# VachaLab/gorder

Hardware: AMD Instinct MI355X
Metric: trajectory frames/sec (higher is better)
Workload: dtype f32

## Files before the change

gorder_amd/csrc/gorder_hip.hip:

```cpp
#include <hip/hip_runtime.h>

#include <dlfcn.h>

#include <cmath>
#include <cstdio>
#include <cstdlib>
#include <cstring>
#include <mutex>
#include <new>
#include <string>
#include <deque>
#include <type_traits>
#include <vector>

#include "../../include/gorder_hip.h"
#include "gm_math.h"
#include "plan.h"
#include "collect_store.h"
#include "device_mem.h"
#include "replay_rows.h"
#include "leaflet_rows.h"
#include "timewise_blocks.h"
#include "ordermap_final.h"
#include "order_route.h"
// ... 107 lines not shown
    uint32_t rows_frames = 0;
    RepAcc acc;
    size_t lds_bytes = 0;
    bool direct = false;
    bool force_direct = false;
    uint32_t forced_subrange = 0;
    uint64_t row_bytes = gorder::kClassRowBytes;
    bool on() const { return n_classes != 0; }
};

struct gorder_hip_handle {
    void *traj_cache = nullptr;
    void (*traj_cache_free)(gorder_hip_handle *) = nullptr;
    Plan plan;
    gorder_tables_t tables{};
    int device = 0;
    Stream own_stream;
    hipStream_t stream = nullptr;
    DBuf<Tile> d_tiles;
    DBuf<Item> d_items;
    DBuf<uint32_t> d_tile_slots;
    DBuf<DirectItem> d_direct;
    DBuf<Tile> d_ua_tiles;
    DBuf<gorder::UaItem> d_ua_items;
    DBuf<uint32_t> d_ua_tile_slots;
    uint32_t map_nx = 0, map_ny = 0;
    DBuf<u64> d_map_sums, d_map_cnts;
    DBuf<u64> d_map_packed;
    DBuf<u64> d_map_rec;
    DBuf<gorder::MapRun> d_ua_runs, d_runs;
    DBuf<uint32_t> d_ua_run_begin, d_run_begin;
    DBuf<Item> d_items_by_slot;
    DBuf<uint32_t> d_ua_item_run, d_item_run;
    DBuf<uint4> d_lgrid;
    DBuf<LocalRowPre> d_lrowpre;
    DBuf<LocalEdge> d_ledge;
    DBuf<float4> d_lfinfo;
    static constexpr uint32_t kDecidePause = 16;
    DBuf<uint32_t> d_lsummary;
    HBuf<uint32_t> h_lsummary;
    Event lsummary_written;
    bool lsummary_pending = false;
    uint32_t decide_pause = 0;
    uint64_t decide_submits = 0, decide_paused_submits = 0;
    DBuf<uint32_t> d_lneed;
    DBuf<uint2> d_ltodo;
    size_t map_lds_bytes = 0;
    bool map_staged = false;
    uint64_t map_pending = 0;
    uint64_t map_fold_limit = kMapFoldLimit;
    uint32_t map_max_mol = 1;
    DBuf<u64> d_tw_sums, d_tw_cnts;
    uint64_t tw_cap = 0;
    DBuf<u64> d_twx_blocks, d_twx_rows, d_twx_totals, d_twx_edge;
    DBuf<uint32_t> d_twx_groups;
    DBuf<float> d_twx_out;
    DBuf<uint32_t> d_omx_groups;
    DBuf<float> d_omx_out;
    ExtraArgs extra{};
    DBuf<uint32_t> d_geom_group;
    DBuf<float> d_shapes;
    DBuf<float> d_inv_box;
    uint32_t dyn_slab = 4, local_slab = 4;
    bool local_halo = false;
    size_t local_rec_stride = 0;
    DBuf<XtcCheckpoint> d_xtc_cp;
// ... 536 lines not shown
                           b.aflags, b.arow, h->d_tiles, bond_items(h, s.route), h->d_tile_slots, nt);
    }); });
    return GORDER_OK;
}

int launch_dist(gorder_hip_handle *h, const SubRange &s, const ExtraArgs &e) {
    const uint32_t nt = (uint32_t)h->plan.tiles.size();
    const gorder::FrameChunks c = gorder::dist_chunks(s.nf(), nt, h->wg_target, h->wg_capacity, h->hist_direct ? 0u : (uint32_t)h->hist_table_words,
                                                      h->hist_samples_per_word, kDistChunkMax);
    FrameArgs b = s.frames(c);
    DistArgs da{};
    da.n_edges = h->hist_edges; da.edges = h->d_hist_edges; da.rep = h->hist.rep; da.n_rep = h->hist.n_rep;
    const size_t lds = kDistEdgeBytes + std::max<size_t>(kDistReduceBytes, h->hist_direct ? 0u : h->hist_table_words * sizeof(uint32_t));
    TIMING_MARK(h, s.route.label);
    with_bool(literal_cosine(h), [&](auto AC) { with_bool(h->hist_direct, [&](auto DIRECT) {
        hipLaunchKernelGGL((k_bonds_dist<AC(), DIRECT()>), dim3(nt * c.n_chunks), dim3(kBlock), lds, h->stream, b, e, da, b.xyz, b.box9,
                           b.aflags, b.arow, h->d_tiles, bond_items(h, s.route), h->d_tile_slots, nt);
    }); });
    return GORDER_OK;
}

int launch_extras(gorder_hip_handle *h, const SubRange &s, const ExtraArgs &e) {
    const uint32_t nt = (uint32_t)h->plan.tiles.size();
    const gorder::FrameChunks c = gorder::extras_chunks(s.nf(), nt, h->wg_target, h->wg_capacity, s.route.map_accumulate, false);
    FrameArgs b = s.frames(c);
    TIMING_MARK(h, s.route.label);
    with_bool(literal_cosine(h), [&](auto AC) { with_bool(s.route.maps_only, [&](auto MO) {
        hipLaunchKernelGGL((k_bonds_extras<AC(), MO()>), dim3(nt * c.n_chunks), dim3(kBlock), 0, h->stream, b, e, b.xyz, b.box9, b.aflags,
                           b.arow, h->d_tiles, bond_items(h, s.route), h->d_tile_slots, nt);
    }); });
    return GORDER_OK;
}

int launch_tiled_out(gorder_hip_handle *h, const SubRange &s, const ExtraArgs &e) {
    const gorder::OrderRoute &route = s.route;
    const uint32_t nt = (uint32_t)h->plan.tiles.size();
    const gorder::FrameChunks c = gorder::extras_chunks(s.nf(), nt, h->wg_target, h->wg_capacity, route.map_accumulate,
                                                        route.family == gorder::BondFamily::TiledTw);
    FrameArgs b = s.frames(c);
    const dim3 g(nt * c.n_chunks), blk(kBlock);
    const Item *items = bond_items(h, route);
    TIMING_MARK(h, route.label);
    with_npf(route.npf, [&](auto NPF) { with_bool(b.pbc, [&](auto PBC) { with_bool(b.leaflets, [&](auto LF) { with_axis(h->axis, [&](auto AX) {
        if (route.family == gorder::BondFamily::TiledMaps)
            hipLaunchKernelGGL((k_bonds_tiled_maps<NPF(), PBC(), LF(), AX()>), g, blk, h->lds_bytes, h->stream, b, e, b.xyz,
                               b.box9, b.aflags, b.arow, h->d_tiles, items, h->d_tile_slots, nt, h->lw);
        else with_bool(route.tw_maps, [&](auto MAPS) { with_bool(route.mom, [&](auto MOM) {
            if constexpr (!MOM() || (LF() && !MAPS()))
                hipLaunchKernelGGL((k_bonds_tiled_tw<NPF(), PBC(), LF(), AX(), MAPS(), MOM()>), g, blk, h->lds_bytes, h->stream, b, e,
                                   b.xyz, b.box9, b.aflags, b.arow, h->d_tiles, items, h->d_tile_slots, nt, h->lw);
        }); });
    }); }); }); });
    return GORDER_OK;
}

int launch_map_accumulate(gorder_hip_handle *h, const SubRange &s, uint32_t rec_stride, const gorder::MapRun *runs,
                          const uint32_t *run_begin, uint32_t per_item) {
    const uint32_t n_acc = h->plan.n_acc;
    const uint32_t planes = h->tables.leaflets.method != GORDER_LEAFLETS_NONE ? 2u : 1u;
    const uint32_t ntm = h->map_nx * h->map_ny, n_words = planes * ntm;
    const char *ev = getenv("GORDER_HIP_MAP_CHUNKS");
    const gorder::FrameChunks m = gorder::map_chunks(s.nf(), n_acc, ev ? (uint32_t)std::max(1, atoi(ev)) : 0u);
    TIMING_MARK(h, "k_map_accumulate");
    hipLaunchKernelGGL(k_map_accumulate, dim3(n_acc * m.n_chunks), dim3(1024), n_words * sizeof(unsigned long long), h->stream,
                       h->d_map_rec, runs, run_begin, n_acc, s.nf(), rec_stride, m.frames_per_chunk, per_item, n_words, ntm,
                       h->d_map_packed, n_acc);
    return GORDER_OK;
}

int launch_bond_pass(gorder_hip_handle *h, const SubRange &s, ExtraArgs &e) {
    using gorder::BondFamily;
    e.item_run = h->d_item_run;
    switch (s.route.family) {
    case BondFamily::Classes: ST_TRY(launch_classes(h, s)); break;
    case BondFamily::Shells: ST_TRY(launch_shells(h, s, e)); break;
    case BondFamily::Dist: ST_TRY(launch_dist(h, s, e)); break;
    case BondFamily::Extras: ST_TRY(launch_extras(h, s, e)); break;
    default: ST_TRY(launch_tiled_out(h, s, e)); break;
    }
    if (s.route.map_accumulate) ST_TRY(launch_map_accumulate(h, s, e.rec_stride, h->d_runs, h->d_run_begin, 1u));
    HIP_TRY(h, hipGetLastError());
    return GORDER_OK;
}

int launch_ua_dist(gorder_hip_handle *h, const SubRange &s, const ExtraArgs &e) {
    const uint32_t nt = (uint32_t)h->plan.ua_tiles.size();
    const gorder::FrameChunks c = gorder::dist_chunks(s.nf(), nt, h->wg_target, h->wg_capacity, h->hist_direct ? 0u : (uint32_t)h->hist_table_words,
                                                      h->hist_samples_per_word, kDistChunkMax);
    FrameArgs b = s.frames(c);
    DistArgs da{};
    da.n_edges = h->hist_edges; da.edges = h->d_hist_edges; da.rep = h->hist.rep; da.n_rep = h->hist.n_rep;
    const size_t lds = kDistEdgeBytes + std::max<size_t>(kUaSumBytes, h->hist_direct ? 0u : h->hist_table_words * sizeof(uint32_t));
    const dim3 g((uint32_t)ua_grid(nt, c.n_chunks)), blk(kBlock);
    TIMING_MARK(h, "k_ua_dist");
    with_bool(literal_cosine(h), [&](auto AC) { with_bool(h->hist_direct, [&](auto DIRECT) {
        hipLaunchKernelGGL((k_ua_dist<AC(), DIRECT()>), g, blk, lds, h->stream, b, e, da, b.xyz, b.box9, b.aflags, b.arow, h->d_ua_tiles,
                           h->d_ua_items, h->d_ua_tile_slots, nt);
    }); });
    HIP_TRY(h, hipGetLastError());
    return GORDER_OK;
}

int launch_ua_pass(gorder_hip_handle *h, const SubRange &s, ExtraArgs &e) {
    const gorder::OrderRoute &route = s.route;
    if (route.ua_kernel == gorder::UaKernel::Dist) return launch_ua_dist(h, s, e);
// ... 717 lines not shown
    h->tables = *t;
    h->tables.molecule_types = nullptr;
    h->tables.leaflets.membrane = nullptr;
    h->device = t->device;
    HIP_TRY(h, hipSetDevice(h->device));
    if ((t->flags & GORDER_FLAG_UA_FAST_NORMALISE) && (t->flags & GORDER_FLAG_TRIG_ACOS_COS))
        return fail(h, GORDER_ERR_INVALID_ARGUMENT, "GORDER_FLAG_UA_FAST_NORMALISE (tolerance-bounded) and GORDER_FLAG_TRIG_ACOS_COS (literal) exclude each other");
    if ((t->flags & GORDER_FLAG_CLUSTER_CUTOFF) && t->leaflets.method != GORDER_LEAFLETS_CLUSTERING)
        return fail(h, GORDER_ERR_INVALID_ARGUMENT, "GORDER_FLAG_CLUSTER_CUTOFF needs leaflets.method == GORDER_LEAFLETS_CLUSTERING");
    const bool ua_rows_only = t->timewise && !t->ordermap.enabled && t->geometry.kind == GORDER_GEOM_NONE && !t->dynamic_normal.enabled;
    const int st = gorder::build_plan(*t, env_flag("GORDER_HIP_FORCE_DIRECT"), h->plan, !env_flag("GORDER_HIP_UA_SLOT_WAVES") && !ua_rows_only);
    if (st != GORDER_OK) return fail(h, st, "invalid bond tables");
    const Plan &p = h->plan;
    for (uint32_t m = 0; m < t->n_molecule_types; m++)
        h->map_max_mol = std::max(h->map_max_mol, t->molecule_types[m].n_molecules);
    HIP_TRY(h, h->own_stream.create());
    h->stream = h->own_stream;
    ST_TRY(upload(h, h->d_tiles, p.tiles));
    ST_TRY(upload(h, h->d_items, p.items));
    ST_TRY(upload(h, h->d_tile_slots, p.tile_slots));
    ST_TRY(upload(h, h->d_direct, p.direct));
    ST_TRY(upload(h, h->d_ua_tiles, p.ua_tiles));
    ST_TRY(upload(h, h->d_ua_items, p.ua_items));
    ST_TRY(upload(h, h->d_ua_tile_slots, p.ua_tile_slots));
    ExtraArgs &e = h->extra;
    e.sin_tet = sinf(1.910633f); e.cos_tet = cosf(1.910633f);
    e.sin_ch3 = sinf(2.0943952f); e.cos_ch3 = cosf(2.0943952f);
    e.sin_half = sinf(0.9553165f); e.cos_half = cosf(0.9553165f);
    ST_TRY(create_ordermaps(h, t));
    e.tw = t->timewise ? 1 : 0;
    if (t->timewise && !p.tiles.empty()) {
        if (!h->d_items_by_slot) ST_TRY(upload(h, h->d_items_by_slot, p.items_by_slot));
        ST_TRY(upload(h, h->d_item_run, p.item_run));
    }
    ST_TRY(create_geometry(h, t));
    if ((e.maps || e.tw || e.geom_kind) && !p.direct.empty())
        return fail(h, GORDER_ERR_INVALID_ARGUMENT, "ordermaps / timewise / geometry need every bond to fit an atom window");
    ST_TRY(create_accumulators(h));
    {
        const float *n = t->normal;
        h->n2sq = (n[0] * n[0] + n[1] * n[1]) + n[2] * n[2];
        h->n2 = sqrtf(h->n2sq);
        for (int d = 0; d < 3; d++)
            if (n[d] == 1.0f && n[(d + 1) % 3] == 0.0f && n[(d + 2) % 3] == 0.0f) h->axis = d;
        h->extra.axis = h->axis;
    }
    if (const char *e = getenv("GORDER_HIP_KERNEL")) h->use_gather = strcmp(e, "gather") == 0;
    h->shell_force_direct = env_flag("GORDER_HIP_RADIAL_DIRECT");
    h->hist_force_direct = env_flag("GORDER_HIP_DIST_DIRECT");
    h->nb.force_direct = env_flag("GORDER_HIP_NB_DIRECT");
    if (const char *ev = getenv("GORDER_HIP_NB_SUBRANGE")) h->nb.forced_subrange = (uint32_t)std::max(0, atoi(ev));
    if (const char *ev = getenv("GORDER_HIP_NB_ROW_BYTES")) {
        const long long v = atoll(ev);
        if (v > 0) h->nb.row_bytes = (uint64_t)v;
    }
    if (const char *ev = getenv("GORDER_HIP_CORR_SUBRANGE")) h->corr.forced_subrange = (uint32_t)std::max(0, atoi(ev));
    if (const char *ev = getenv("GORDER_HIP_CORR_GRID")) h->corr.chunk_major = strcmp(ev, "chunks") == 0;
    if (const char *ev = getenv("GORDER_HIP_DIST_SAMPLES_PER_WORD")) h->hist_samples_per_word = (uint32_t)std::min(std::max(0, atoi(ev)), 1 << 16);
    if (const char *e = getenv("GORDER_HIP_MOL_ROWS_STAGING")) {
        const long long v = atoll(e);
        if (v > 0) h->mol_stage_bytes = (size_t)v;
    }
    if (const char *e = getenv("GORDER_HIP_WG_TARGET")) {
        const int w = atoi(e);
        if (w > 0) h->wg_target = (uint32_t)w;
    }
// ... 533 lines not shown
    ri.bond_tiles = !p.tiles.empty(); ri.ua_tiles = !p.ua_tiles.empty(); ri.direct_items = !p.direct.empty(); ri.ua_fast_flag = (h->tables.flags & GORDER_FLAG_UA_FAST_NORMALISE) != 0;
    ri.global_leaflets = h->tables.leaflets.method == GORDER_LEAFLETS_GLOBAL; ri.spec_enabled = h->spec_enabled && !h->corr.on(); ri.have_assignment = h->have_assignment;
    ri.shells = h->n_shells != 0;
    ri.dist = h->hist_edges != 0;
    ri.classes = h->nb.on();
    ri.mol_rows = h->mol.n_groups != 0 && !h->mol_failed;
    ri.ua_samples_flag = (h->tables.flags & GORDER_FLAG_UA_SAMPLES) != 0;
    ri.npf5 = env_flag("GORDER_HIP_NPF5"); ri.tw_gather = env_flag("GORDER_HIP_TW_GATHER"); ri.maps_gather = env_flag("GORDER_HIP_MAPS_GATHER");
    ri.every_frame_assigns = b.aframes.size() == b.n_frames;
    b.route = gorder::choose_order_route(ri);
    if (!b.route.speculative) return;
    spec_poll(h, false);
    const uint32_t slot = (uint32_t)(h->spec_batches % gorder_hip_handle::kSpecRing);
    if (h->spec_ring_frames[slot]) (void)hipEventSynchronize(h->spec_counters_copied[slot]), spec_poll(h, false);
    ri.spec_enabled = h->spec_enabled && !h->corr.on();
    if (!ri.spec_enabled) b.route = gorder::choose_order_route(ri);
}

static int fill_flag_rows(gorder_hip_handle *h, Batch &b) {
    if (!b.leaflets) return GORDER_OK;
    const bool spec = b.route.speculative;
    if (spec) std::fill(b.arow.begin(), b.arow.end(), 0u);
    const size_t rows = (b.ltable ? b.replay.expand.size() : b.aframes.size()) + 1;
    ST_TRY(ensure_flag_rows(h, rows, rows + rows / 4, true));
    ST_TRY(upload_if_changed(h, h->d_arow, h->up_arow, h->up_arow_valid, b.arow));
    if (h->collect & GORDER_COLLECT_LEAFLETS)
        for (uint32_t f : b.aframes) b.collect_frames.push_back(b.frame_index[f]);
    if (spec) b.spec_aframes = b.aframes;
    else if (b.ltable) BATCH_TRY(replay_flag_rows(h, b.replay));
    else BATCH_TRY(run_leaflets(h, b.d_xyz, b.d_box, b.aframes, 1));
    h->have_assignment = true;
    h->assignment_frame = b.last_assign_frame;
    b.n_new_rows = spec ? 0 : (b.ltable ? b.replay.expand.size() : b.aframes.size());
    return GORDER_OK;
}

static int grow_frame_rows(gorder_hip_handle *h, const Batch &b) {
    if (!h->extra.tw || h->n_frames + b.n_frames <= h->tw_cap) return GORDER_OK;
    const size_t row = 3 * (size_t)h->plan.n_acc;
    const uint64_t ncap = (h->n_frames + b.n_frames) * 2;
    DBuf<u64> ns, nc;
    ST_TRY(allocate(h, ns, ncap * row));
    ST_TRY(allocate(h, nc, ncap * row));
    HIP_TRY(h, hipMemsetAsync(ns, 0, ncap * row * sizeof(u64), h->stream));
    HIP_TRY(h, hipMemsetAsync(nc, 0, ncap * row * sizeof(u64), h->stream));
    if (h->d_tw_sums) {
        HIP_TRY(h, hipMemcpyAsync(ns, h->d_tw_sums, h->n_frames * row * sizeof(u64), hipMemcpyDeviceToDevice, h->stream));
        HIP_TRY(h, hipMemcpyAsync(nc, h->d_tw_cnts, h->n_frames * row * sizeof(u64), hipMemcpyDeviceToDevice, h->stream));
        HIP_TRY(h, hipStreamSynchronize(h->stream));
    }
    h->d_tw_sums.swap(ns); h->d_tw_cnts.swap(nc); h->tw_cap = ncap;
    return GORDER_OK;
}

static int set_batch_normals(gorder_hip_handle *h, Batch &b) {
    const Plan &p = h->plan;
    FrameArgs &a = b.a;
    a.xyz = b.d_xyz; a.box9 = b.d_box; a.n_atoms = p.n_atoms; a.n_frames = b.n_frames;
    a.pbc = b.pbc ? 1 : 0;
    a.nx = h->tables.normal[0]; a.ny = h->tables.normal[1]; a.nz = h->tables.normal[2]; a.n2 = h->n2; a.n2sq = h->n2sq;
    a.leaflets = b.leaflets ? 1 : 0; a.aflags = h->d_aflags; a.arow = h->d_arow; a.n_mol_total = p.n_mol_total;
    a.acc = h->d_acc; a.rep = h->d_rep; a.n_rep = h->n_rep; a.n_acc = p.n_acc; a.err = h->d_err;
    h->manual_active = false;
    if (h->manual_frames) {
        const size_t n4 = (size_t)b.n_frames * p.n_mol_total;
        BATCH_TRY(ensure(h, h->d_dyn_normals, n4));
// ... 1318 lines not shown
```

gorder_amd/csrc/kernels_extras.h:

```cpp
#pragma once

namespace {

struct ExtraArgs {
    int maps;
    uint32_t plane;
    float x0, y0, binx, biny;
    uint32_t nx, ny;
    unsigned long long *map_packed;
    unsigned long long *map_rec;
    const uint32_t *item_run;
    uint32_t rec_frame0, rec_stride;
    const float4 *dyn;
    int bin_core;
    float inv_binx, inv_biny;
    int axis;
    int tw;
    unsigned long long *tw_sums;
    unsigned long long *tw_cnts;
    unsigned long long tw_row0;
    float sin_tet, cos_tet, sin_ch3, cos_ch3, sin_half, cos_half;
    int geom_kind, geom_invert, geom_orient;
    float geom_thr;
    const float *shapes;
    const float *inv_box;
    uint8_t *touched;
};

__device__ __forceinline__ bool geom_inside(const ExtraArgs &e, const float *sh, float px, float py, float pz,
                                            const float *box, bool pbc, int &bad) {
    bool in = true;
    if (e.geom_kind == GORDER_GEOM_CUBOID) {
        float x = px - sh[0], y = py - sh[1], z = pz - sh[2];
        if (pbc) {
            x = gm_wrap(x, box[0], bad); y = gm_wrap(y, box[1], bad); z = gm_wrap(z, box[2], bad);
            in = (x <= sh[3]) && (y <= sh[4]) && (z <= sh[5]);
        } else {
            in = (x >= 0.0f) && (x <= sh[3]) && (y >= 0.0f) && (y <= sh[4]) && (z >= 0.0f) && (z <= sh[5]);
        }
    } else if (e.geom_kind == GORDER_GEOM_CYLINDER) {
        const int o = e.geom_orient;
        const float dx = px - sh[0], dy = py - sh[1], dz = pz - sh[2];
        float x = o == 0 ? dx : (o == 1 ? dy : dz), da = o == 0 ? dy : (o == 1 ? dz : dx), db = o == 0 ? dz : (o == 1 ? dx : dy);
        if (pbc) {
            const float bo = o == 0 ? box[0] : (o == 1 ? box[1] : box[2]), ba = o == 0 ? box[1] : (o == 1 ? box[2] : box[0]),
                        bb = o == 0 ? box[2] : (o == 1 ? box[0] : box[1]);
            da = gm_min_image(da, ba, bad); db = gm_min_image(db, bb, bad); x = gm_wrap(x, bo, bad);
        }
        in = (da * da + db * db < e.geom_thr) && (pbc ? true : (x >= 0.0f)) && (x <= sh[7]);
    } else {
        float dx = px - sh[0], dy = py - sh[1], dz = pz - sh[2];
        if (pbc) { dx = gm_min_image(dx, box[0], bad); dy = gm_min_image(dy, box[1], bad); dz = gm_min_image(dz, box[2], bad); }
        in = (dx * dx + dy * dy) + dz * dz < e.geom_thr;
// ... 220 lines not shown
        __syncthreads();
        if (f0 + G < f_full) S::template load<false>(a, t, f0 + G, f_end, sk, si, pre);
        if (active) S::template compute<1>(a, t, it, f0, lds, lw, acc, bad, nan_which, nan_frame, &mo);
        rec_store(e, tile_id, f0, tid, words);
        __syncthreads();
    }
    if (f_full < f_end) {
        S::template load<true>(a, t, f_full, f_end, sk, si, pre);
        S::template store<true>(a, t, f_full, f_end, sk, si, pre, lds, lw);
        __syncthreads();
#pragma unroll
        for (uint32_t m = 0; m < kRecFrames; m++) words[m] = kMapNoSample;
        if (active) S::template compute_tail<1>(a, t, it, f_full, f_end, lds, lw, acc, bad, nan_which, nan_frame, &mo);
        rec_store(e, tile_id, f_full, tid, words);
        __syncthreads();
    }
    raise_tile_errors(a.err, tc, tile_slots, nan_which, nan_frame, bad);
    __syncthreads();
    fold_tile_sums(a.rep, a.n_rep, a.n_acc, tc, acc, lds, [&] { return tile_slots[tc.t.slot0 + tc.tid]; });
}

template <int NPF, bool PBC, bool LEAF, int AXIS, bool MAPS, bool MOM = false>
__global__ __launch_bounds__(kBlock, 4) void k_bonds_tiled_tw(FrameArgs a_in, ExtraArgs e, const float *__restrict__ xyz,
                                                             const float *__restrict__ box9, const uint8_t *__restrict__ aflags,
                                                             const uint32_t *__restrict__ arow, const Tile *__restrict__ tiles,
                                                             const Item *__restrict__ items, const uint32_t *__restrict__ tile_slots,
                                                             uint32_t n_tiles, uint32_t lw) {
    constexpr int G = (int)kRecFrames;
    extern __shared__ __attribute__((aligned(16))) float lds[];
    __shared__ int l_tick[kRecFrames][kBlock];
    __shared__ uint8_t l_side[kRecFrames][kBlock];
    __shared__ uint32_t l_slot_run[kBlock];
    __shared__ uint32_t l_slot_id[kBlock];
    using S = TiledStage<G, NPF, false, PBC, LEAF, AXIS>;
    FrameArgs a = a_in;
    a.xyz = xyz; a.box9 = box9; a.aflags = aflags; a.arow = arow;
    const uint32_t tile_id = blockIdx.x % n_tiles, chunk = blockIdx.x / n_tiles;
    const Tile t = tiles[tile_id];
    const uint32_t tid = threadIdx.x;
    const uint32_t sk = tid / S::TPF, si = tid % S::TPF;
    const bool active = tid < t.n_items;
    Item it{0, 0, 0, 0, 0};
    if (active) {
        it = items[t.item0 + tid];
        const uint32_t run = e.item_run[t.item0 + tid];
        if ((run >> 16) == tid) l_slot_run[it.lslot] = run;
    }
    const uint32_t f_begin = a.frame0 + chunk * a.frames_per_chunk;
    const uint32_t f_end = min(a.n_frames, f_begin + a.frames_per_chunk);
    const TileCtx tc{t, it, tile_id, chunk, tid, active, f_begin, f_end};
    unsigned long long words[kRecFrames], mwords[MAPS ? kRecFrames : 1];
    TiledMapOut mo{};
    if (MAPS) {
        mo = tiled_map_out(e, mwords);
        mo.ticks = words;
    } else {
        mo.nx = 0;
        mo.words = words;
    }
    SampleAcc acc;
    int bad = 0;
    uint32_t nan_which = 0, nan_frame = kNoNan;
    v4f pre[NPF];
    const uint32_t my_slot = tid < t.n_slots ? tile_slots[t.slot0 + tid] : 0u;
    l_slot_id[tid] = my_slot;
    uint2 own = make_uint2(0u, 0u), my_head = make_uint2(0u, 0xffffffffu);
    if (MOM) {
        own = a.own[tile_id];
        const uint32_t hq = a.own_head_begin[tile_id] + (tid & 63u);
        if (hq < a.own_head_begin[tile_id + 1u]) my_head = a.own_heads[hq];
    }
    if (f_begin + G <= f_end) S::template load<false>(a, t, f_begin, f_end, sk, si, pre);
    for (uint32_t fs = f_begin; fs < f_end; fs += G) {
        const bool full = fs + G <= f_end;
        bool finite;
        if (full) {
            finite = S::template store<false, MOM>(a, t, fs, f_end, sk, si, pre, lds, lw);
        } else {
            S::template load<true>(a, t, fs, f_end, sk, si, pre);
            finite = S::template store<true, MOM>(a, t, fs, f_end, sk, si, pre, lds, lw);
        }
        __syncthreads();
        if (full && fs + 2u * G <= f_end) S::template load<false>(a, t, fs + G, f_end, sk, si, pre);
        if (MOM && fs + sk < f_end) {
            static_assert(!MOM || (uint32_t)G * 64u == kBlock, "a wave per frame slot");
            tiled_moments(a, t, own, tile_id, n_tiles, fs + sk, lds + (size_t)sk * lw, finite, my_head);
        }
#pragma unroll
        for (uint32_t k = 0; k < kRecFrames; k++) { words[k] = kMapNoSample; if (MAPS) mwords[k] = kMapNoSample; }
        if (active) {
            if (full) S::template compute<MAPS ? 3 : 2>(a, t, it, fs, lds, lw, acc, bad, nan_which, nan_frame, &mo);
            else S::template compute_tail<MAPS ? 3 : 2>(a, t, it, fs, f_end, lds, lw, acc, bad, nan_which, nan_frame, &mo);
        }
        if constexpr (MAPS) rec_store(e, tile_id, fs, tid, mwords);
#pragma unroll
        for (uint32_t k = 0; k < kRecFrames; k++) {
            l_tick[k][tid] = (int)(uint32_t)words[k];
            l_side[k][tid] = words[k] == kMapNoSample ? (uint8_t)2 : (uint8_t)(words[k] >> 32);
        }
        __syncthreads();
        for (uint32_t w = tid; w < kRecFrames * t.n_slots; w += kBlock) {
            const uint32_t k = w % kRecFrames, ls = w / kRecFrames;
            if (fs + k >= f_end) continue;
            const uint32_t run = l_slot_run[ls], tid0 = run >> 16, n = run & 0xffffu;
            int s_all = 0, s_low = 0;
            uint32_t n_all = 0, n_low = 0;
            for (uint32_t j = 0; j < n; j++) {
                const uint32_t side = l_side[k][tid0 + j];
                const int tick = l_tick[k][tid0 + j];
                if (side == 2u) continue;
                s_all += tick; n_all += 1u;
                if (side == 1u) { s_low += tick; n_low += 1u; }
            }
            if (!n_all) continue;
            const uint32_t slot = l_slot_id[ls];
            const size_t row = ((size_t)e.tw_row0 + fs + k) * 3u * a.n_acc;
            atomicAdd(&e.tw_sums[row + slot], (unsigned long long)(long long)s_all);
            atomicAdd(&e.tw_cnts[row + slot], (unsigned long long)n_all);
            if (LEAF) {
                const uint32_t n_up = n_all - n_low;
                if (n_up) {
                    atomicAdd(&e.tw_sums[row + (size_t)a.n_acc + slot], (unsigned long long)(long long)(s_all - s_low));
                    atomicAdd(&e.tw_cnts[row + (size_t)a.n_acc + slot], (unsigned long long)n_up);
                }
            }
        }
    }
    __syncthreads();
    raise_tile_errors(a.err, tc, tile_slots, nan_which, nan_frame, bad);
    fold_tile_sums(a.rep, a.n_rep, a.n_acc, tc, acc, lds, [&] { return my_slot; });
}

constexpr uint32_t kMapRunBatch = 1024;
__global__ __launch_bounds__(1024) void k_map_accumulate(const unsigned long long *__restrict__ rec,
                                                         const gorder::MapRun *__restrict__ runs,
                                                         const uint32_t *__restrict__ run_begin, uint32_t n_slots,
                                                         uint32_t rec_frames, uint32_t rec_stride,
                                                         uint32_t frames_per_chunk, uint32_t k_max,
                                                         uint32_t n_words , uint32_t n_tiles_map,
                                                         unsigned long long *__restrict__ map_packed, uint32_t n_acc) {
    extern __shared__ unsigned long long l_map[];
    typedef unsigned long long ull2 __attribute__((ext_vector_type(2)));
    const uint32_t slot = blockIdx.x % n_slots, chunk = blockIdx.x / n_slots;
    const uint32_t r0 = run_begin[slot], r1 = run_begin[slot + 1];
    if (r0 == r1) return;
    const uint32_t f0 = chunk * frames_per_chunk, f1 = min(rec_frames, f0 + frames_per_chunk);
    for (uint32_t w = threadIdx.x; w < n_words; w += blockDim.x) l_map[w] = 0ull;
    __syncthreads();
    auto add = [&](unsigned long long v) {
        if (v != kMapNoSample) atomicAdd(&l_map[(uint32_t)(v >> 32)], kMapOne + (unsigned long long)(long long)(int)(uint32_t)v);
    };
    if (k_max == 1u) {
        __shared__ uint32_t l_pref[kMapRunBatch + 1];
        const uint32_t fb0 = f0 / kRecFrames, fb1 = (f1 + kRecFrames - 1) / kRecFrames;
        for (uint32_t rb = r0; rb < r1; rb += kMapRunBatch) {
            const uint32_t nr = min(kMapRunBatch, r1 - rb);
            for (uint32_t i = threadIdx.x; i < nr; i += blockDim.x) l_pref[i + 1u] = runs[rb + i].n;
// ... 79 lines not shown
```

gorder_amd/csrc/kernels_timewise.h:

```cpp
#pragma once

using gorder::kTwChunkFrames;
typedef unsigned long long tw_u64;

__device__ __forceinline__ float tw_mean(tw_u64 sum, tw_u64 count) {
    const long long q = (long long)sum / (long long)count;
    return (float)((double)q / 1e6);
}

__global__ __launch_bounds__(256) void k_tw_blocks(const tw_u64 *__restrict__ tw_sums, const tw_u64 *__restrict__ tw_cnts,
                                                   uint32_t row_words, uint32_t fold_words, tw_u64 n_used, tw_u64 first_position,
                                                   tw_u64 block_size, tw_u64 *__restrict__ out_sums, tw_u64 *__restrict__ out_cnts) {
    const uint32_t j = blockIdx.y * blockDim.x + threadIdx.x;
    if (j >= fold_words) return;
    tw_u64 r = (tw_u64)blockIdx.x * kTwChunkFrames;
    const tw_u64 end = r + kTwChunkFrames < n_used ? r + kTwChunkFrames : n_used;
    while (r < end) {
        const tw_u64 b = gorder::tw_block_of(first_position, r, block_size);
        const tw_u64 e = gorder::tw_segment_end(first_position, r, end, b, block_size);
        tw_u64 s = 0, c = 0;
        for (tw_u64 q = r; q < e; q++) {
            s += tw_sums[q * row_words + j];
            c += tw_cnts[q * row_words + j];
        }
        atomicAdd(&out_sums[b * row_words + j], s);
        atomicAdd(&out_cnts[b * row_words + j], c);
        r = e;
    }
}

__global__ __launch_bounds__(256) void k_tw_lower(tw_u64 *__restrict__ sums, tw_u64 *__restrict__ cnts, uint32_t n_acc, tw_u64 n) {
    const tw_u64 i = (tw_u64)blockIdx.x * 256u + threadIdx.x;
    if (i >= n) return;
    const tw_u64 at = (i / n_acc) * 3u * n_acc + i % n_acc;
    sums[at + 2u * n_acc] = sums[at] - sums[at + n_acc];
    cnts[at + 2u * n_acc] = cnts[at] - cnts[at + n_acc];
}

__global__ __launch_bounds__(64) void k_tw_errors(const tw_u64 *__restrict__ block_sums, const tw_u64 *__restrict__ block_cnts,
                                                  uint32_t n_blocks, uint32_t n_acc, const uint32_t *__restrict__ group_begin,
                                                  const uint32_t *__restrict__ slots, float *__restrict__ errors) {
    const uint32_t g = blockIdx.x / 3u, w = blockIdx.x % 3u, lane = threadIdx.x;
    const uint32_t m0 = group_begin[g], m1 = group_begin[g + 1];
    float mean = 0.0f, var = 0.0f;
    bool empty = false;
    for (int pass = 0; pass < 2; pass++) {
        for (uint32_t b = 0; b < n_blocks; b++) {
            const tw_u64 *bs = block_sums + ((tw_u64)b * 3u + w) * n_acc, *bc = block_cnts + ((tw_u64)b * 3u + w) * n_acc;
            tw_u64 s = 0, c = 0;
            for (uint32_t m = m0 + lane; m < m1; m += 64u) { s += bs[slots[m]]; c += bc[slots[m]]; }
            s = wave_sum_rows(s);
            c = wave_sum_rows(c);
            if (c == 0) { empty = true; continue; }
            const float x = tw_mean(s, c);
            if (pass == 0) mean = mean + x;
            else { const float d = mean - x; var = var + d * d; }
        }
        if (pass == 0) mean = mean / (float)n_blocks;
    }
    if (lane == 0) errors[blockIdx.x] = empty ? __builtin_nanf("") : sqrtf(var / (float)(n_blocks - 1u));
}

__global__ __launch_bounds__(256) void k_tw_group_rows(const tw_u64 *__restrict__ tw_sums, const tw_u64 *__restrict__ tw_cnts,
                                                       uint32_t n_acc, int leaflets, tw_u64 n_frames, uint32_t n_groups,
                                                       const uint32_t *__restrict__ group_begin, const uint32_t *__restrict__ slots,
                                                       tw_u64 *__restrict__ rows_sums, tw_u64 *__restrict__ rows_cnts) {
    const uint32_t lane = threadIdx.x & 63u;
    const tw_u64 item = (tw_u64)blockIdx.x * 4u + (uint32_t)__builtin_amdgcn_readfirstlane((int)(threadIdx.x >> 6));
    if (item >= n_frames * n_groups) return;
// ... 87 lines not shown
```

gorder_amd/csrc/plan.h:

```cpp
#pragma once
#include <algorithm>
#include <map>
#include <tuple>
#include <cstdint>
#include <utility>
#include <vector>

#include "../../include/gorder_hip.h"

namespace gorder {

#ifndef GORDER_BLOCK
#define GORDER_BLOCK 256
#endif
constexpr uint32_t kBlock = GORDER_BLOCK;
constexpr uint32_t kMaxWindow = 1024;

struct Item {
    uint16_t li, lj;
    uint16_t lslot;
    uint16_t pad;
    uint32_t mol;
};
struct Tile {
// ... 1 lines not shown
    uint32_t item0, n_items;
    uint32_t slot0, n_slots;
};
struct DirectItem {
    uint32_t i, j, slot, mol;
};
struct UaItem {
    uint16_t l[4];
    uint16_t lslot0;
    uint16_t kind;
    uint32_t mol;
};

struct MapRun {
    uint32_t tile, tid0, n, k;
};

struct Plan {
    uint32_t n_atoms = 0, n_acc = 0, n_mol_total = 0;
    uint32_t max_window = 0;
    std::vector<Tile> tiles;
    std::vector<Item> items;
    std::vector<uint32_t> tile_slots;
    std::vector<DirectItem> direct;
    std::vector<Tile> ua_tiles;
    std::vector<UaItem> ua_items;
    std::vector<uint32_t> ua_tile_slots;
    std::vector<MapRun> ua_runs;
    std::vector<uint32_t> ua_run_begin;
    std::vector<Item> items_by_slot;
    std::vector<uint32_t> item_run, ua_item_run;
    std::vector<MapRun> runs;
    std::vector<uint32_t> run_begin;
    std::vector<uint32_t> mol0;
    std::vector<uint32_t> slot0;
    bool spec_ok = false;
    std::vector<uint32_t> own;
    std::vector<uint32_t> own_head_begin;
    std::vector<uint32_t> own_heads;
};

struct Sample {
    uint32_t i, j, slot, mol;
};
struct UaSample {
    uint32_t a[4];
    uint32_t slot0, kind, mol, type;
};

inline uint32_t bank_conflict_cycles(const Item *items, uint32_t n) {
    uint32_t extra = 0;
    for (uint32_t h = 0; h < n; h += 32u)
        for (int which = 0; which < 2; which++) {
            uint16_t seen[32][8];
            uint32_t cnt[32] = {0};
            uint32_t worst = 1;
            for (uint32_t q = h; q < std::min(n, h + 32u); q++) {
                const uint16_t at = which ? items[q].lj : items[q].li;
                uint32_t &c = cnt[at % 32u];
                bool dup = false;
                for (uint32_t k = 0; k < std::min(c, 8u); k++) dup = dup || seen[at % 32u][k] == at;
                if (!dup) { if (c < 8u) seen[at % 32u][c] = at; c++; }
                worst = std::max(worst, c);
            }
            extra += worst - 1u;
        }
// ... 3 lines not shown
    constexpr uint32_t kHalf = 32;
    if (n <= kHalf) return;
    const uint32_t n_bins = (n + kHalf - 1) / kHalf;
    auto cap = [&](uint32_t b) { return b + 1 < n_bins ? kHalf : n - kHalf * (n_bins - 1); };
    struct Bin {
        std::vector<uint16_t> at_i[kHalf], at_j[kHalf];
        std::vector<Item> got;
    };
    std::vector<Bin> bins(n_bins);
    auto added = [](const std::vector<uint16_t> &v, uint16_t a) {
        return (!v.empty() && std::find(v.begin(), v.end(), a) == v.end()) ? 1u : 0u;
    };
    for (uint32_t q = 0; q < n; q++) {
        const Item it = items[q];
        uint32_t best = n_bins, best_cost = ~0u;
        size_t best_fill = 0;
        for (uint32_t b = 0; b < n_bins; b++) {
            Bin &bin = bins[b];
            if (bin.got.size() >= cap(b)) continue;
            const uint32_t cost = added(bin.at_i[it.li % kHalf], it.li) + added(bin.at_j[it.lj % kHalf], it.lj);
            if (cost < best_cost || (cost == best_cost && bin.got.size() > best_fill)) {
                best = b; best_cost = cost; best_fill = bin.got.size();
            }
        }
        Bin &bin = bins[best];
        auto note = [](std::vector<uint16_t> &v, uint16_t a) { if (std::find(v.begin(), v.end(), a) == v.end()) v.push_back(a); };
        note(bin.at_i[it.li % kHalf], it.li);
        note(bin.at_j[it.lj % kHalf], it.lj);
        bin.got.push_back(it);
    }
    std::vector<Item> order;
    for (uint32_t b = 0; b < n_bins; b++) order.insert(order.end(), bins[b].got.begin(), bins[b].got.end());
    if (5u * bank_conflict_cycles(order.data(), n) <= 4u * bank_conflict_cycles(items, n)) std::copy(order.begin(), order.end(), items);
}

inline int build_plan(const gorder_tables_t &t, bool force_direct, Plan &p, bool ua_quads = true) {
    p = Plan();
    p.n_atoms = t.n_atoms;
    if (t.n_atoms == 0 || (t.n_molecule_types && !t.molecule_types)) return GORDER_ERR_INVALID_ARGUMENT;
    std::vector<Sample> samples;
    std::vector<UaSample> ua_samples;
    uint32_t slot = 0, mol = 0;
    for (uint32_t m = 0; m < t.n_molecule_types; m++) {
        const gorder_moltype_t &mt = t.molecule_types[m];
        p.mol0.push_back(mol);
        p.slot0.push_back(slot);
        if (mt.n_bond_types && !mt.bonds) return GORDER_ERR_INVALID_ARGUMENT;
        for (uint32_t bt = 0; bt < mt.n_bond_types; bt++) {
            for (uint32_t k = 0; k < mt.n_molecules; k++) {
                const uint32_t *b = mt.bonds + 2 * ((size_t)bt * mt.n_molecules + k);
                if (b[0] >= t.n_atoms || b[1] >= t.n_atoms || b[0] == b[1]) return GORDER_ERR_INVALID_ARGUMENT;
                samples.push_back({b[0], b[1], slot + bt, mol + k});
            }
        }
        slot += mt.n_bond_types;
        if (mt.n_ua_atoms && !mt.ua_atoms) return GORDER_ERR_INVALID_ARGUMENT;
        for (uint32_t a = 0; a < mt.n_ua_atoms; a++) {
            const uint32_t kind = mt.ua_atoms[a].kind;
            if (kind < GORDER_UA_CH1_SAT || kind > GORDER_UA_CH1_UNSAT || !mt.ua_atoms[a].indices)
                return GORDER_ERR_INVALID_ARGUMENT;
            const uint32_t nidx = kind == GORDER_UA_CH1_SAT ? 4u : 3u;
            for (uint32_t k = 0; k < mt.n_molecules; k++) {
                const uint32_t *ix = mt.ua_atoms[a].indices + 4 * (size_t)k;
                UaSample us{{ix[0], ix[1], ix[2], nidx == 4 ? ix[3] : ix[1]}, slot, kind, mol + k, m};
                for (uint32_t q = 0; q < nidx; q++)
                    if (ix[q] >= t.n_atoms) return GORDER_ERR_INVALID_ARGUMENT;
// ... 222 lines not shown
                    for (uint32_t q = 0; q < nt[0].n_items; q++) {
                        p.items[nt[0].item0 + q].li = (uint16_t)(p.items[nt[0].item0 + q].li + shift0);
                        p.items[nt[0].item0 + q].lj = (uint16_t)(p.items[nt[0].item0 + q].lj + shift0);
                    }
                p.tiles = nt;
                p.max_window = std::max(p.max_window, widest);
                p.own = own;
                p.spec_ok = true;
            }
        }
    }
    {
        p.items_by_slot = p.items;
        std::vector<std::pair<uint32_t, MapRun>> run_of_slot;
        for (uint32_t ti = 0; ti < p.tiles.size(); ti++) {
            const Tile &tile = p.tiles[ti];
            std::stable_sort(p.items_by_slot.begin() + tile.item0, p.items_by_slot.begin() + tile.item0 + tile.n_items,
                             [](const Item &x, const Item &y) { return x.lslot < y.lslot; });
            p.item_run.resize((size_t)tile.item0 + tile.n_items, 0u);
            for (uint32_t i = 0; i < tile.n_items;) {
                const uint16_t ls = p.items_by_slot[tile.item0 + i].lslot;
                uint32_t n = 1;
                while (i + n < tile.n_items && p.items_by_slot[tile.item0 + i + n].lslot == ls) n++;
                run_of_slot.push_back({p.tile_slots[tile.slot0 + ls], MapRun{ti, i, n, 0}});
                for (uint32_t j = 0; j < n; j++) p.item_run[tile.item0 + i + j] = (i << 16) | n;
                i += n;
            }
        }
        std::stable_sort(run_of_slot.begin(), run_of_slot.end(),
                         [](const std::pair<uint32_t, MapRun> &x, const std::pair<uint32_t, MapRun> &y) { return x.first < y.first; });
        p.run_begin.assign((size_t)p.n_acc + 1, 0);
        for (const auto &r : run_of_slot) { p.run_begin[r.first + 1]++; p.runs.push_back(r.second); }
        for (uint32_t sl = 0; sl < p.n_acc; sl++) p.run_begin[sl + 1] += p.run_begin[sl];
    }
    return GORDER_OK;
}

inline int selfcheck_plan(const gorder_tables_t &t, const Plan &p) {
    std::vector<Sample> want, got;
    uint32_t slot = 0, mol = 0;
    for (uint32_t m = 0; m < t.n_molecule_types; m++) {
        const gorder_moltype_t &mt = t.molecule_types[m];
        for (uint32_t bt = 0; bt < mt.n_bond_types; bt++)
            for (uint32_t k = 0; k < mt.n_molecules; k++) {
                const uint32_t *b = mt.bonds + 2 * ((size_t)bt * mt.n_molecules + k);
                want.push_back({b[0], b[1], slot + bt, mol + k});
            }
        slot += mt.n_bond_types;
        for (uint32_t a = 0; a < mt.n_ua_atoms; a++) {
            const uint32_t kind = mt.ua_atoms[a].kind;
            slot += kind == GORDER_UA_CH3 ? 3 : kind == GORDER_UA_CH2 ? 2 : 1;
        }
        mol += mt.n_molecules;
    }
    for (const Tile &tile : p.tiles) {
        if (tile.n_items == 0 || tile.n_items > kBlock) return 1;
        if (tile.n_window == 0 || tile.n_window > kMaxWindow) return 2;
        if ((uint64_t)tile.atom0 + tile.n_window > t.n_atoms) return 3;
        if (tile.n_slots == 0 || tile.n_slots > tile.n_items) return 4;
        for (uint32_t q = 0; q < tile.n_items; q++) {
            const Item &it = p.items[tile.item0 + q];
            if (it.li >= tile.n_window || it.lj >= tile.n_window || it.lslot >= tile.n_slots) return 5;
            got.push_back({tile.atom0 + it.li, tile.atom0 + it.lj, p.tile_slots[tile.slot0 + it.lslot], it.mol});
        }
    }
    for (const DirectItem &d : p.direct) got.push_back({d.i, d.j, d.slot, d.mol});
    auto cmp = [](const Sample &a, const Sample &b) {
        if (a.slot != b.slot) return a.slot < b.slot;
        if (a.mol != b.mol) return a.mol < b.mol;
        if (a.i != b.i) return a.i < b.i;
        return a.j < b.j;
    };
    std::sort(want.begin(), want.end(), cmp);
    std::sort(got.begin(), got.end(), cmp);
    if (want.size() != got.size()) return 6;
    for (size_t q = 0; q < want.size(); q++)
        if (want[q].i != got[q].i || want[q].j != got[q].j || want[q].slot != got[q].slot ||
            want[q].mol != got[q].mol)
            return 7;
    if (p.items_by_slot.size() != p.items.size() || p.run_begin.size() != (size_t)p.n_acc + 1) return 8;
    std::vector<uint32_t> covered(p.items.size(), 0);
    for (uint32_t sl = 0; sl < p.n_acc; sl++)
        for (uint32_t r = p.run_begin[sl]; r < p.run_begin[sl + 1]; r++) {
            const MapRun &run = p.runs[r];
            if (run.tile >= p.tiles.size() || run.k != 0 || run.tid0 + run.n > p.tiles[run.tile].n_items) return 9;
            const Tile &tile = p.tiles[run.tile];
            for (uint32_t j = 0; j < run.n; j++) {
                const Item &it = p.items_by_slot[tile.item0 + run.tid0 + j];
                if (p.tile_slots[tile.slot0 + it.lslot] != sl) return 10;
                if (p.item_run.size() != p.items.size() || p.item_run[tile.item0 + run.tid0 + j] != ((run.tid0 << 16) | run.n))
                    return 16;
                covered[tile.item0 + run.tid0 + j]++;
            }
        }
    for (uint32_t c : covered)
        if (c != 1) return 11;
    if (!p.ua_tiles.empty()) {
        if (p.ua_run_begin.size() != (size_t)p.n_acc + 1) return 12;
        size_t lanes = 0, want_lanes = 0;
        for (const UaItem &it : p.ua_items) want_lanes += it.kind == GORDER_UA_CH3 ? 3 : it.kind == GORDER_UA_CH2 ? 2 : 1;
        for (uint32_t sl = 0; sl < p.n_acc; sl++)
            for (uint32_t r = p.ua_run_begin[sl]; r < p.ua_run_begin[sl + 1]; r++) {
                const MapRun &run = p.ua_runs[r];
                if (run.tile >= p.ua_tiles.size() || run.k > 2 || run.tid0 + run.n > p.ua_tiles[run.tile].n_items) return 13;
                const Tile &tile = p.ua_tiles[run.tile];
                for (uint32_t j = 0; j < run.n; j++) {
                    const UaItem &it = p.ua_items[tile.item0 + run.tid0 + j];
                    if (p.ua_tile_slots[tile.slot0 + it.lslot0 + run.k] != sl) return 14;
                    if (p.ua_item_run.size() != p.ua_items.size() ||
                        p.ua_item_run[tile.item0 + run.tid0 + j] != ((run.tid0 << 16) | run.n))
                        return 17;
                    lanes++;
                }
            }
        if (lanes != want_lanes) return 15;
    }
    return 0;
}

}
```

Measured before the change: 20.89 million.

## Precompute timewise per-frame counts from plan and per-row leaflet upper counts

```diff
diff --git a/gorder_amd/csrc/gorder_hip.hip b/gorder_amd/csrc/gorder_hip.hip
--- a/gorder_amd/csrc/gorder_hip.hip
+++ b/gorder_amd/csrc/gorder_hip.hip
@@ -163,6 +163,10 @@
     DBuf<uint32_t> d_ua_run_begin, d_run_begin;
     DBuf<Item> d_items_by_slot;
     DBuf<uint32_t> d_ua_item_run, d_item_run;
+    DBuf<uint32_t> d_tw_count_add;
+    DBuf<uint32_t> d_tw_mol_begin, d_tw_slot_type, d_tw_upper;
+    uint32_t tw_flag_rows = 1;
+    bool tw_upper_made = false;
     DBuf<uint4> d_lgrid;
     DBuf<LocalRowPre> d_lrowpre;
     DBuf<LocalEdge> d_ledge;
@@ -765,7 +769,21 @@
     return GORDER_OK;
 }
 
-int launch_tiled_out(gorder_hip_handle *h, const SubRange &s, const ExtraArgs &e) {
+int launch_upper_counts(gorder_hip_handle *h, ExtraArgs &e) {
+    const uint32_t n_types = (uint32_t)h->plan.mol0.size();
+    const size_t words = (size_t)h->tw_flag_rows * n_types;
+    if (!h->tw_upper_made) {
+        if (words > 0x7fffffffull) return fail(h, GORDER_ERR_INVALID_ARGUMENT, "per-frame rows: too many flag rows in one batch");
+        ST_TRY(ensure(h, h->d_tw_upper, words));
+        hipLaunchKernelGGL(k_tw_upper_counts, dim3((uint32_t)words), dim3(64), 0, h->stream, (const uint8_t *)h->d_aflags, h->plan.n_mol_total,
+                           (const uint32_t *)h->d_tw_mol_begin, n_types, (uint32_t *)h->d_tw_upper);
+        h->tw_upper_made = true;
+    }
+    e.tw_upper = h->d_tw_upper; e.tw_slot_type = h->d_tw_slot_type; e.tw_n_types = n_types;
+    return GORDER_OK;
+}
+
+int launch_tiled_out(gorder_hip_handle *h, const SubRange &s, ExtraArgs &e) {
     const gorder::OrderRoute &route = s.route;
     const uint32_t nt = (uint32_t)h->plan.tiles.size();
     const gorder::FrameChunks c = gorder::extras_chunks(s.nf(), nt, h->wg_target, h->wg_capacity, route.map_accumulate,
@@ -774,6 +792,7 @@
     const dim3 g(nt * c.n_chunks), blk(kBlock);
     const Item *items = bond_items(h, route);
     TIMING_MARK(h, route.label);
+    if (route.family == gorder::BondFamily::TiledTw && b.leaflets) ST_TRY(launch_upper_counts(h, e));
     with_npf(route.npf, [&](auto NPF) { with_bool(b.pbc, [&](auto PBC) { with_bool(b.leaflets, [&](auto LF) { with_axis(h->axis, [&](auto AX) {
         if (route.family == gorder::BondFamily::TiledMaps)
             hipLaunchKernelGGL((k_bonds_tiled_maps<NPF(), PBC(), LF(), AX()>), g, blk, h->lds_bytes, h->stream, b, e, b.xyz,
@@ -804,6 +823,7 @@
 int launch_bond_pass(gorder_hip_handle *h, const SubRange &s, ExtraArgs &e) {
     using gorder::BondFamily;
     e.item_run = h->d_item_run;
+    e.tw_count_add = h->d_tw_count_add;
     switch (s.route.family) {
     case BondFamily::Classes: ST_TRY(launch_classes(h, s)); break;
     case BondFamily::Shells: ST_TRY(launch_shells(h, s, e)); break;
@@ -1587,6 +1607,15 @@
     if (t->timewise && !p.tiles.empty()) {
         if (!h->d_items_by_slot) ST_TRY(upload(h, h->d_items_by_slot, p.items_by_slot));
         ST_TRY(upload(h, h->d_item_run, p.item_run));
+        ST_TRY(upload(h, h->d_tw_count_add, p.tw_count_add));
+        if (t->leaflets.method != GORDER_LEAFLETS_NONE) {
+            std::vector<uint32_t> mol_begin = p.mol0, slot_type(p.n_acc, 0u);
+            mol_begin.push_back(p.n_mol_total);
+            for (uint32_t m = 0; m < p.slot0.size(); m++)
+                for (uint32_t sl = p.slot0[m]; sl < (m + 1 < p.slot0.size() ? p.slot0[m + 1] : p.n_acc); sl++) slot_type[sl] = m;
+            ST_TRY(upload(h, h->d_tw_mol_begin, mol_begin));
+            ST_TRY(upload(h, h->d_tw_slot_type, slot_type));
+        }
     }
     ST_TRY(create_geometry(h, t));
     if ((e.maps || e.tw || e.geom_kind) && !p.direct.empty())
@@ -2186,6 +2215,8 @@
     h->have_assignment = true;
     h->assignment_frame = b.last_assign_frame;
     b.n_new_rows = spec ? 0 : (b.ltable ? b.replay.expand.size() : b.aframes.size());
+    h->tw_flag_rows = (uint32_t)b.n_new_rows + 1u;
+    h->tw_upper_made = false;
     return GORDER_OK;
 }
 
diff --git a/gorder_amd/csrc/kernels_extras.h b/gorder_amd/csrc/kernels_extras.h
--- a/gorder_amd/csrc/kernels_extras.h
+++ b/gorder_amd/csrc/kernels_extras.h
@@ -19,6 +19,9 @@
     unsigned long long *tw_sums;
     unsigned long long *tw_cnts;
     unsigned long long tw_row0;
+    const uint32_t *tw_count_add;
+    const uint32_t *tw_upper, *tw_slot_type;
+    uint32_t tw_n_types;
     float sin_tet, cos_tet, sin_ch3, cos_ch3, sin_half, cos_half;
     int geom_kind, geom_invert, geom_orient;
     float geom_thr;
@@ -305,6 +308,8 @@
     __shared__ uint8_t l_side[kRecFrames][kBlock];
     __shared__ uint32_t l_slot_run[kBlock];
     __shared__ uint32_t l_slot_id[kBlock];
+    __shared__ uint32_t l_slot_own[kBlock];
+    __shared__ uint32_t l_slot_type[LEAF ? kBlock : 1];
     using S = TiledStage<G, NPF, false, PBC, LEAF, AXIS>;
     FrameArgs a = a_in;
     a.xyz = xyz; a.box9 = box9; a.aflags = aflags; a.arow = arow;
@@ -337,6 +342,8 @@
     v4f pre[NPF];
     const uint32_t my_slot = tid < t.n_slots ? tile_slots[t.slot0 + tid] : 0u;
     l_slot_id[tid] = my_slot;
+    l_slot_own[tid] = tid < t.n_slots ? e.tw_count_add[t.slot0 + tid] : 0u;
+    if constexpr (LEAF) l_slot_type[tid] = tid < t.n_slots ? e.tw_slot_type[my_slot] : 0u;
     uint2 own = make_uint2(0u, 0u), my_head = make_uint2(0u, 0xffffffffu);
     if (MOM) {
         own = a.own[tile_id];
@@ -385,17 +392,20 @@
                 s_all += tick; n_all += 1u;
                 if (side == 1u) { s_low += tick; n_low += 1u; }
             }
-            if (!n_all) continue;
             const uint32_t slot = l_slot_id[ls];
             const size_t row = ((size_t)e.tw_row0 + fs + k) * 3u * a.n_acc;
+            const uint32_t known = l_slot_own[ls];
+            const unsigned long long c_all = (unsigned long long)known + (unsigned long long)((long long)n_all - (long long)n);
+            if (c_all) atomicAdd(&e.tw_cnts[row + slot], c_all);
+            if (LEAF && known) {
+                const uint32_t n_upper = e.tw_upper[(size_t)a.arow[fs + k] * e.tw_n_types + l_slot_type[ls]];
+                if (n_upper) atomicAdd(&e.tw_cnts[row + (size_t)a.n_acc + slot], (unsigned long long)n_upper);
+            }
+            if (!n_all) continue;
             atomicAdd(&e.tw_sums[row + slot], (unsigned long long)(long long)s_all);
-            atomicAdd(&e.tw_cnts[row + slot], (unsigned long long)n_all);
             if (LEAF) {
-                const uint32_t n_up = n_all - n_low;
-                if (n_up) {
+                if (n_all - n_low)
                     atomicAdd(&e.tw_sums[row + (size_t)a.n_acc + slot], (unsigned long long)(long long)(s_all - s_low));
-                    atomicAdd(&e.tw_cnts[row + (size_t)a.n_acc + slot], (unsigned long long)n_up);
-                }
             }
         }
     }
diff --git a/gorder_amd/csrc/kernels_timewise.h b/gorder_amd/csrc/kernels_timewise.h
--- a/gorder_amd/csrc/kernels_timewise.h
+++ b/gorder_amd/csrc/kernels_timewise.h
@@ -35,6 +35,17 @@
     const tw_u64 at = (i / n_acc) * 3u * n_acc + i % n_acc;
     sums[at + 2u * n_acc] = sums[at] - sums[at + n_acc];
     cnts[at + 2u * n_acc] = cnts[at] - cnts[at + n_acc];
+}
+
+__global__ __launch_bounds__(64) void k_tw_upper_counts(const uint8_t *__restrict__ aflags, uint32_t n_mol_total,
+                                                        const uint32_t *__restrict__ mol_begin, uint32_t n_types,
+                                                        uint32_t *__restrict__ U) {
+    const uint32_t type = blockIdx.x % n_types, row = blockIdx.x / n_types;
+    const uint8_t *flags = aflags + (size_t)row * n_mol_total;
+    uint32_t n = 0;
+    for (uint32_t m = mol_begin[type] + threadIdx.x; m < mol_begin[type + 1]; m += 64u) n += flags[m] == 0 ? 1u : 0u;
+    n = wave_sum_rows(n);
+    if (threadIdx.x == 0) U[blockIdx.x] = n;
 }
 
 __global__ __launch_bounds__(64) void k_tw_errors(const tw_u64 *__restrict__ block_sums, const tw_u64 *__restrict__ block_cnts,
diff --git a/gorder_amd/csrc/plan.h b/gorder_amd/csrc/plan.h
--- a/gorder_amd/csrc/plan.h
+++ b/gorder_amd/csrc/plan.h
@@ -57,6 +57,7 @@
     std::vector<uint32_t> item_run, ua_item_run;
     std::vector<MapRun> runs;
     std::vector<uint32_t> run_begin;
+    std::vector<uint32_t> tw_count_add;
     std::vector<uint32_t> mol0;
     std::vector<uint32_t> slot0;
     bool spec_ok = false;
@@ -126,6 +127,23 @@
     std::vector<Item> order;
     for (uint32_t b = 0; b < n_bins; b++) order.insert(order.end(), bins[b].got.begin(), bins[b].got.end());
     if (5u * bank_conflict_cycles(order.data(), n) <= 4u * bank_conflict_cycles(items, n)) std::copy(order.begin(), order.end(), items);
+}
+
+template <class LocalSlot>
+inline std::vector<uint32_t> known_row_counts(const std::vector<Tile> &tiles, size_t n_tile_slots, const std::vector<MapRun> &runs,
+                                              const std::vector<uint32_t> &run_begin, LocalSlot lslot_of) {
+    std::vector<uint32_t> add(n_tile_slots, 0u);
+    for (size_t sl = 0; sl + 1 < run_begin.size(); sl++) {
+        if (run_begin[sl] == run_begin[sl + 1]) continue;
+        const MapRun *owner = &runs[run_begin[sl]];
+        uint32_t total = 0;
+        for (uint32_t r = run_begin[sl]; r < run_begin[sl + 1]; r++) {
+            total += runs[r].n;
+            if (runs[r].tile < owner->tile) owner = &runs[r];
+        }
+        add[tiles[owner->tile].slot0 + lslot_of(*owner)] = total;
+    }
+    return add;
 }
 
 inline int build_plan(const gorder_tables_t &t, bool force_direct, Plan &p, bool ua_quads = true) {
@@ -414,6 +432,9 @@
         p.run_begin.assign((size_t)p.n_acc + 1, 0);
         for (const auto &r : run_of_slot) { p.run_begin[r.first + 1]++; p.runs.push_back(r.second); }
         for (uint32_t sl = 0; sl < p.n_acc; sl++) p.run_begin[sl + 1] += p.run_begin[sl];
+        p.tw_count_add = known_row_counts(p.tiles, p.tile_slots.size(), p.runs, p.run_begin, [&](const MapRun &r) {
+            return (uint32_t)p.items_by_slot[p.tiles[r.tile].item0 + r.tid0].lslot;
+        });
     }
     return GORDER_OK;
 }
@@ -477,6 +498,22 @@
         }
     for (uint32_t c : covered)
         if (c != 1) return 11;
+    if (p.tw_count_add.size() != p.tile_slots.size()) return 18;
+    std::vector<uint32_t> owners(p.n_acc, 0), holders(p.n_acc, 0);
+    std::vector<uint64_t> owned(p.n_acc, 0);
+    for (const Tile &tile : p.tiles)
+        for (uint32_t ls = 0; ls < tile.n_slots; ls++) {
+            const uint32_t sl = p.tile_slots[tile.slot0 + ls], add = p.tw_count_add[tile.slot0 + ls];
+            if (sl >= p.n_acc || (add != 0) != (holders[sl] == 0)) return 19;
+            holders[sl]++;
+            owners[sl] += add != 0;
+            owned[sl] += add;
+        }
+    for (uint32_t sl = 0; sl < p.n_acc; sl++) {
+        uint64_t run_sum = 0;
+        for (uint32_t r = p.run_begin[sl]; r < p.run_begin[sl + 1]; r++) run_sum += p.runs[r].n;
+        if (owners[sl] != (run_sum ? 1u : 0u) || owned[sl] != run_sum) return 20;
+    }
     if (!p.ua_tiles.empty()) {
         if (p.ua_run_begin.size() != (size_t)p.n_acc + 1) return 12;
         size_t lanes = 0, want_lanes = 0;
```

Measured after the change: 20.66 million. -1.1%, worse.
